# CEA-LIST/runia_core

Measured on AMD Instinct MI355X. Metric: OOD scores/sec, LaREM 16-MC PCA-256 (ResNet-18 layer4 latent 512x4x4), higher is better.
Workload: dtype f64

## Files before the change

include/runia_hip.h:

```cpp
#ifndef RUNIA_HIP_H
#define RUNIA_HIP_H

#include <stddef.h>
#include <stdint.h>

#ifdef __cplusplus
extern "C" {
#endif

#define RUNIA_OK 0
#define RUNIA_E_INVALID (-1)
#define RUNIA_E_LAUNCH (-2)
#define RUNIA_E_NODEVICE (-3)
#define RUNIA_E_WORKSPACE (-4)

typedef void* runia_stream_t;

int runia_abi_version(void);
const char* runia_error_string(int code);
int runia_device_count(void);
int runia_clock_probe(uint64_t* out4, int chain, runia_stream_t stream);
int runia_time_next_launch(void* start_event, void* stop_event);

int runia_mc_stack_f32(const float* x, const float* rand, int64_t rand_image_stride, float* out,
// ... 71 lines not shown

int runia_row_lse_msp_f32(const float* logits, float* lse, float* msp, int64_t N, int64_t C,
                          runia_stream_t stream);

int runia_l2_normalize_f32(const float* x, float* y, int64_t N, int64_t D, runia_stream_t stream);
size_t runia_knn_workspace_bytes(int64_t N, int64_t M, int64_t D, int k);
int runia_knn_piece_products(int64_t N, int64_t M, int64_t D);
size_t runia_knn_bank_state_bytes(int64_t M, int64_t D);
int runia_knn_prepare_bank_f32(const float* bank, void* state, size_t state_bytes, int64_t M, int64_t D,
                               runia_stream_t stream);
size_t runia_knn_prepared_workspace_bytes(int64_t N, int64_t M, int64_t D, int k);
int runia_knn_kth_prepared_f32(const float* q, const float* bank, const void* state, size_t state_bytes, float* score,
                               void* workspace, size_t workspace_bytes, int64_t N, int64_t M, int64_t D, int k,
                               runia_stream_t stream);
int runia_knn_kth_f32(const float* q, const float* bank, float* score, void* workspace,
                      size_t workspace_bytes, int64_t N, int64_t M, int64_t D, int k,
                      runia_stream_t stream);

int runia_kde_score_f64(const double* train, const double* x, double* score, int64_t M, int64_t N,
                        int64_t D, double bandwidth, runia_stream_t stream);
int runia_kde_score_kernel_f64(const double* train, const double* x, double* score, int64_t M, int64_t N, int64_t D,
                               double bandwidth, int kind, runia_stream_t stream);
int runia_row_sqnorm_f64(const double* x, double* out, int64_t N, int64_t D, runia_stream_t stream);
size_t runia_kde_workspace_bytes(int64_t N, int64_t M);
int runia_kde_score_packed_f64(const double* packed_train_t, const double* train_sqnorm, const double* x,
                               double* score, void* workspace, size_t workspace_bytes, int64_t M, int64_t N,
                               int64_t D, double bandwidth, runia_stream_t stream);

int runia_mc_entropy_supported(int H, int W, int n_mc, int k);
size_t runia_mc_entropy_workspace_bytes(int64_t N, int H, int W, int n_mc);
int runia_mc_mask_table_f32(const float* rand, int64_t rand_image_stride, void* workspace,
                            size_t workspace_bytes, int64_t N, int H, int W, int n_mc, double drop_prob,
                            int block_size, runia_stream_t stream);
int runia_mc_stack_table_f32(const float* x, const float* rand, int64_t rand_image_stride, float* z,
                             void* workspace, size_t workspace_bytes, int64_t N, int C, int H, int W, int n_mc,
                             double drop_prob, int block_size, runia_stream_t stream);
int runia_mc_entropy_from_table_f32(const float* x, const void* workspace, size_t workspace_bytes, double* h,
                                    float* z_out, double* zero_fill, int64_t N, int C, int H, int W, int n_mc,
                                    int k, double min_dist, runia_stream_t stream);
int runia_mc_entropy_f32(const float* x, const float* rand, int64_t rand_image_stride, double* h,
                         float* z_out, double* zero_fill, void* workspace, size_t workspace_bytes, int64_t N,
                         int C, int H, int W, int n_mc, double drop_prob, int block_size, int k, double min_dist,
                         runia_stream_t stream);
int runia_mc_draws_f32(float* out, int64_t N, int n_mc, int H, int W, uint64_t seed, int64_t first_image,
                       runia_stream_t stream);
int runia_mc_mask_table_counter_f32(uint64_t seed, int64_t first_image, void* workspace, size_t workspace_bytes,
                                    int64_t N, int H, int W, int n_mc, double drop_prob, int block_size,
                                    int redraw_dead_layers, runia_stream_t stream);
int runia_mc_entropy_counter_f32(const float* x, uint64_t seed, int64_t first_image, double* h, float* z_out,
                                 double* zero_fill, void* workspace, size_t workspace_bytes, int64_t N, int C, int H,
                                 int W, int n_mc, double drop_prob, int block_size, int k, double min_dist,
                                 int redraw_dead_layers, runia_stream_t stream);
int runia_pca_md_score_f64(const double* h, const double* packed_ct, const double* bias,
                           const double* scale, const double* md_mean, const double* packed_p,
                           double* score, double* y_out, int64_t N, int64_t D, int64_t n,
                           runia_stream_t stream);
size_t runia_proj_sq_workspace_bytes(int64_t N);
int runia_proj_sq_accumulate_f64(const double* h, const double* packed_m, const double* c, double* score,
                                 int64_t N, int64_t D, int64_t r, runia_stream_t stream);
int runia_proj_sq_score_f64(const double* h, const double* packed_m, const double* c, double* score,
                            void* workspace, size_t workspace_bytes, int64_t N, int64_t D, int64_t r,
                            runia_stream_t stream);
int runia_proj_sq_accumulate_trap_f64(const double* h, const double* packed_m, const double* c, double* score,
                                      int64_t N, int64_t D, int64_t r, runia_stream_t stream);
int runia_proj_sq_score_trap_f64(const double* h, const double* packed_m, const double* c, double* score,
                                 void* workspace, size_t workspace_bytes, int64_t N, int64_t D, int64_t r,
// ... 245 lines not shown
```

runia_core_amd/_hip.py:

```python
from __future__ import annotations

import contextlib
import ctypes
import os
import threading
from ctypes import c_char_p, c_double, c_float, c_int, c_int64, c_size_t, c_uint64, c_void_p
from typing import NamedTuple, Optional, Tuple, Union

import numpy as np
import torch

from . import config as _config

_LIB_PATH = os.path.join(os.path.dirname(os.path.abspath(__file__)), "librunia_hip.so")
_lib: Optional[ctypes.CDLL] = None

_SIGNATURES = {
    "runia_abi_version": (c_int, []),
    "runia_error_string": (c_char_p, [c_int]),
    "runia_device_count": (c_int, []),
    "runia_clock_probe": (c_int, [c_void_p, c_int, c_void_p]),
    "runia_time_next_launch": (c_int, [c_void_p, c_void_p]),
    "runia_mc_stack_f32": (
        c_int,
# ... 41 lines not shown
        c_int,
        [c_void_p, c_void_p, c_void_p, c_void_p, c_void_p, c_void_p, c_size_t, c_int64, c_int64, c_int, c_void_p],
    ),
    "runia_mahalanobis_score_f64": (
        c_int,
        [c_void_p, c_void_p, c_void_p, c_void_p, c_void_p, c_void_p, c_size_t, c_int64, c_int64, c_int, c_void_p],
    ),
    "runia_row_lse_msp_f32": (c_int, [c_void_p, c_void_p, c_void_p, c_int64, c_int64, c_void_p]),
    "runia_l2_normalize_f32": (c_int, [c_void_p, c_void_p, c_int64, c_int64, c_void_p]),
    "runia_kde_score_kernel_f64": (c_int, [c_void_p, c_void_p, c_void_p, c_int64, c_int64, c_int64, c_double, c_int, c_void_p]),
    "runia_knn_workspace_bytes": (c_size_t, [c_int64, c_int64, c_int64, c_int]),
    "runia_knn_piece_products": (c_int, [c_int64, c_int64, c_int64]),
    "runia_knn_bank_state_bytes": (c_size_t, [c_int64, c_int64]),
    "runia_knn_prepare_bank_f32": (c_int, [c_void_p, c_void_p, c_size_t, c_int64, c_int64, c_void_p]),
    "runia_knn_prepared_workspace_bytes": (c_size_t, [c_int64, c_int64, c_int64, c_int]),
    "runia_knn_kth_prepared_f32": (c_int, [c_void_p, c_void_p, c_void_p, c_size_t, c_void_p, c_void_p, c_size_t, c_int64, c_int64,
                                           c_int64, c_int, c_void_p]),
    "runia_knn_kth_f32": (
        c_int,
        [c_void_p, c_void_p, c_void_p, c_void_p, c_size_t, c_int64, c_int64, c_int64, c_int, c_void_p],
    ),
    "runia_kde_score_f64": (c_int, [c_void_p, c_void_p, c_void_p, c_int64, c_int64, c_int64, c_double, c_void_p]),
    "runia_row_sqnorm_f64": (c_int, [c_void_p, c_void_p, c_int64, c_int64, c_void_p]),
    "runia_kde_workspace_bytes": (c_size_t, [c_int64, c_int64]),
    "runia_kde_score_packed_f64": (
        c_int,
        [c_void_p, c_void_p, c_void_p, c_void_p, c_void_p, c_size_t, c_int64, c_int64, c_int64, c_double, c_void_p],
    ),
    "runia_mc_entropy_supported": (c_int, [c_int, c_int, c_int, c_int]),
    "runia_mc_entropy_workspace_bytes": (c_size_t, [c_int64, c_int, c_int, c_int]),
    "runia_mc_mask_table_f32": (
        c_int,
        [c_void_p, c_int64, c_void_p, c_size_t, c_int64, c_int, c_int, c_int, c_double, c_int, c_void_p],
    ),
    "runia_mc_stack_table_f32": (
        c_int,
        [c_void_p, c_void_p, c_int64, c_void_p, c_void_p, c_size_t, c_int64, c_int, c_int, c_int, c_int, c_double, c_int,
         c_void_p],
    ),
    "runia_mc_entropy_from_table_f32": (
        c_int,
        [c_void_p, c_void_p, c_size_t, c_void_p, c_void_p, c_void_p, c_int64, c_int, c_int, c_int, c_int, c_int,
         c_double, c_void_p],
    ),
    "runia_mc_entropy_f32": (
        c_int,
        [c_void_p, c_void_p, c_int64, c_void_p, c_void_p, c_void_p, c_void_p, c_size_t, c_int64, c_int, c_int, c_int,
         c_int, c_double, c_int, c_int, c_double, c_void_p],
    ),
    "runia_mc_draws_f32": (c_int, [c_void_p, c_int64, c_int, c_int, c_int, c_uint64, c_int64, c_void_p]),
    "runia_mc_mask_table_counter_f32": (
        c_int,
        [c_uint64, c_int64, c_void_p, c_size_t, c_int64, c_int, c_int, c_int, c_double, c_int, c_int, c_void_p],
    ),
    "runia_mc_entropy_counter_f32": (
        c_int,
        [c_void_p, c_uint64, c_int64, c_void_p, c_void_p, c_void_p, c_void_p, c_size_t, c_int64, c_int, c_int, c_int,
         c_int, c_double, c_int, c_int, c_double, c_int, c_void_p],
    ),
    "runia_select_hist_f32": (c_int, [c_void_p, c_void_p, c_int64, ctypes.c_uint32, ctypes.c_uint32, c_int, c_void_p]),
    "runia_cholesky_f32": (c_int, [c_void_p, c_void_p, c_int64, c_int64, c_double, c_void_p]),
    "runia_cholesky_f64": (c_int, [c_void_p, c_void_p, c_int64, c_int64, c_double, c_void_p]),
    "runia_gmm_log_prob_workspace_bytes": (c_size_t, [c_int64, c_int64, c_int]),
    "runia_gmm_log_prob_f32": (c_int, [c_void_p, c_void_p, c_void_p, c_void_p, c_void_p, c_void_p, c_void_p, c_size_t, c_int64,
                                       c_int64, c_int, c_void_p]),
    "runia_ood_metrics_workspace_bytes": (c_size_t, [c_int64]),
# ... 1056 lines not shown
def reserve_timed_events(n: int) -> None:
    pool = _TIMED_EVENT_POOL.setdefault(torch.cuda.current_device(), [])
    for _ in range(int(n)):
        e0, e1 = torch.cuda.Event(enable_timing=True), torch.cuda.Event(enable_timing=True)
        e0.record()
        e1.record()
        pool.append((e0, e1))


def _timed_launch_events():
    pool = _TIMED_EVENT_POOL.setdefault(torch.cuda.current_device(), [])
    if not pool:
        reserve_timed_events(1)
    e0, e1 = pool.pop()
    call("runia_time_next_launch", e0.cuda_event, e1.cuda_event)
    return e0, e1


def _timed_call(name: str, *args):
    e0, e1 = _timed_launch_events()
    try:
        launch(name, *args)
    finally:
        load_library().runia_time_next_launch(None, None)
    return e0, e1


def mc_entropy_supported(h: int, w: int, n_mc: int, k: int) -> bool:
    return bool(query("runia_mc_entropy_supported", int(h), int(w), int(n_mc), int(k)))


@_device_guard()
def mc_mask_table(rand: Union[torch.Tensor, CounterDraws, None], n: int, h: int, w: int, n_mc: int, drop_prob: float,
                  block_size: int, out: Optional[torch.Tensor] = None) -> torch.Tensor:
    lib = load_library()
    dev = require_gpu()
    assert 0 < n <= 65535
    ws_bytes = int(lib.runia_mc_entropy_workspace_bytes(n, h, w, n_mc))
    if out is None:
        out = torch.empty(max(ws_bytes, 16), dtype=torch.uint8, device=dev)
    assert out.is_cuda and out.dtype == torch.uint8 and out.numel() >= ws_bytes
    if isinstance(rand, CounterDraws):
        launch("runia_mc_mask_table_counter_f32", int(rand.seed) & (2**64 - 1), int(rand.first_image), out.data_ptr(), ws_bytes,
               n, h, w, n_mc, float(drop_prob), int(block_size), int(bool(rand.redraw_dead_layers)))
        return out
    rand, stride = _draws(rand, n, n_mc, h, w, copy=False)
    launch("runia_mc_mask_table_f32", _ptr(rand), stride, out.data_ptr(), ws_bytes, n, h, w, n_mc,
           float(drop_prob) if rand is not None else 0.0, int(block_size))
    return out


@_device_guard()
def mc_entropy(x: torch.Tensor, rand: Union[torch.Tensor, CounterDraws, None], n_mc: int, drop_prob: float, block_size: int, k: int,
               min_dist: float = 1e-5, want_samples: bool = False, out: Optional[torch.Tensor] = None,
               kernel_events: Optional[list] = None, zero_fill: Optional[torch.Tensor] = None,
               table: Optional[torch.Tensor] = None):
    lib = load_library()
    require_gpu()
    assert x.is_cuda and x.dtype == torch.float32 and x.dim() == 4
    x = x.contiguous()
    n, c, hh, ww = x.shape
    if table is not None:
        h = torch.empty((n, c), dtype=torch.float64, device=x.device) if out is None else out
        assert h.is_cuda and h.dtype == torch.float64 and h.shape == (n, c) and h.is_contiguous()
        z = torch.empty((n * n_mc, c), dtype=torch.float32, device=x.device) if want_samples else None
        ws_bytes = int(lib.runia_mc_entropy_workspace_bytes(n, hh, ww, n_mc))
        assert table.is_cuda and table.numel() >= ws_bytes and n <= 65535
        if zero_fill is not None:
            assert zero_fill.is_cuda and zero_fill.dtype == torch.float64 and zero_fill.shape == (n,) and zero_fill.is_contiguous()
        args = (x.data_ptr(), table.data_ptr(), ws_bytes, h.data_ptr(), _ptr(z), _ptr(zero_fill), n, c, hh, ww, n_mc, int(k),
                float(min_dist))
        if kernel_events is not None:
            kernel_events.append(_timed_call("runia_mc_entropy_from_table_f32", *args))
        else:
            launch("runia_mc_entropy_from_table_f32", *args)
        return (h, z) if want_samples else h
    counter = rand if isinstance(rand, CounterDraws) else None
    rand, stride = _draws(None if counter is not None else rand, n, n_mc, hh, ww)
    if out is None:
        h = torch.empty((n, c), dtype=torch.float64, device=x.device)
    else:
# ... 800 lines not shown
```

runia_core_amd/csrc/fused.hip:

```cpp
#include "common.hpp"
#include "entropy_core.hpp"
#include "mfma_f64_tile.hpp"
#include "philox.hpp"
#include "div_consts.hpp"
#include "trap_order.hpp"

namespace {

using namespace runia_entropy;
using namespace runia_mfma;

constexpr int kMaxMC = 64;
typedef float f2 __attribute__((ext_vector_type(2)));

__device__ __forceinline__ void layer_consts(int cnt, int& m, float& flag, float& zh, float& zl) {
  const int a = cnt ? __ffs(cnt) - 1 : 0;
  m = cnt >> a;
  flag = __uint_as_float((unsigned)(127 - a) << 23);
  zh = cnt ? __uint_as_float(runia_div::kDivHi[(m - 1) >> 1]) : NAN;
  zl = cnt ? __uint_as_float(runia_div::kDivLo[(m - 1) >> 1]) : 0.f;
}

__device__ __forceinline__ float add_f32(float a, float b) {
  float r;
// ... 4 lines not shown
__device__ __forceinline__ float div_newton(float u, float den, float r) {
  const float q = u * r;
  const float e = fmaf(-den, q, u);
  return fmaf(e, r, q);
}

template <int HT, int WT>
__host__ __device__ constexpr int mask_slot(int p) {
  if constexpr (HT % 2 == 0) {
    const int y = p / WT, xw = p - y * WT;
    return ((y >> 1) * WT + xw) * 2 + (y & 1);
  } else {
    return p;
  }
}

template <int HT, int WT>
__host__ __device__ constexpr int slot_position(int slot) {
  if constexpr (HT % 2 == 0) {
    const int e = slot & 1, t = slot >> 1;
    const int k = t / WT, xw = t - k * WT;
    return (2 * k + e) * WT + xw;
  } else {
    return slot;
  }
}

template <int HT, int WT>
__device__ __forceinline__ unsigned long long columns_below(int k) {
  unsigned long long row = (k >= 64) ? ~0ull : ((1ull << k) - 1ull), m = 0ull;
#pragma unroll
  for (int y = 0; y < HT; ++y) m |= row << (y * WT);
  return m;
}

constexpr int kMaskBitsWaves = 4;

template <int HT, int WT, int NP, bool REDRAW = false>
__global__ __launch_bounds__(64 * kMaskBitsWaves) void mc_mask_bits_kernel(const float* __restrict__ rnd,
                                                                           int64_t rand_stride,
                                                                           float* __restrict__ table, int64_t N,
                                                                           int n_mc, float gamma, int block_size,
                                                                           int identity, int sort_layers,
                                                                           uint64_t rng_seed, int64_t first_image) {
  constexpr int HW = HT * WT;
  static_assert(HW <= 64 && NP <= 64, "one drop layer per 64-bit word");
  constexpr bool DIV = (64 % HW == 0);
  constexpr int WORDS = (NP * HW + 63) / 64;
  constexpr unsigned long long FULL = (HW == 64) ? ~0ull : ((1ull << HW) - 1ull);
  const int lane = threadIdx.x & 63;
  const int64_t img = (int64_t)blockIdx.x * kMaskBitsWaves + (threadIdx.x >> 6);
  if (img >= N) return;
  const int bit0 = lane * HW, word0 = bit0 >> 6, off = bit0 & 63;
  const int pad = block_size / 2;

  auto seeds_of = [&](unsigned attempt) -> unsigned long long {
    float d[WORDS];
    if (rnd) {
      const float* r = rnd + img * rand_stride;
#pragma unroll
      for (int t = 0; t < WORDS; ++t) {
        const int i = lane + 64 * t;
        d[t] = (i < n_mc * HW) ? r[i] : 1.0f;
      }
    } else {
#pragma unroll
      for (int q = 0; q < (WORDS + 3) / 4; ++q) {
        const runia_philox::u4 b = runia_philox::lane_block(rng_seed, (uint64_t)(first_image + img), lane, q, attempt);
#pragma unroll
        for (int j = 0; j < 4; ++j) {
          const int t = 4 * q + j;
          if (t < WORDS) d[t] = (lane + 64 * t < n_mc * HW) ? runia_philox::component(b, j) : 1.0f;
        }
      }
    }
    unsigned long long lo = 0ull, hi = 0ull;
#pragma unroll
    for (int t = 0; t < WORDS; ++t) {
      const unsigned long long w = __ballot(d[t] < gamma);
      if (t == word0) lo = w;
      if (!DIV && t == word0 + 1) hi = w;
    }
    unsigned long long sd = lo >> off;
    if (!DIV && off + HW > 64) sd |= hi << (64 - off);
    return sd & FULL;
  };
  auto keep_of = [&](unsigned long long seed) -> unsigned long long {
    unsigned long long hx = 0ull;
    for (int dx = 0; dx < block_size; ++dx) {
      const int ox = dx - pad;
      if (ox >= WT || -ox >= WT) continue;
      hx |= (ox >= 0) ? ((seed >> ox) & columns_below<HT, WT>(WT - ox))
                      : ((seed << -ox) & ~columns_below<HT, WT>(-ox) & FULL);
    }
    unsigned long long dropped = 0ull;
    for (int dy = 0; dy < block_size; ++dy) {
      const int oy = dy - pad;
      if (oy >= HT || -oy >= HT) continue;
      dropped |= (oy >= 0) ? (hx >> (oy * WT)) : ((hx << (-oy * WT)) & FULL);
    }
    return ~dropped & FULL;
  };

  unsigned long long keep = identity ? FULL : keep_of(seeds_of(0u));
  if (REDRAW && !identity && !rnd) {
    for (unsigned attempt = 1; attempt <= 16u; ++attempt) {
      if (__ballot(lane < n_mc && keep == 0ull) == 0ull) break;
      const unsigned long long again = keep_of(seeds_of(attempt));
      if (keep == 0ull) keep = again;
    }
  }
  const int cnt = __popcll(keep);
  int m;
  float flag, zh, zl;
  layer_consts(cnt, m, flag, zh, zl);
  const int key = m ? m : 127;
  int rank = 0;
#pragma unroll
  for (int j = 0; j < NP; ++j) {
    const int o = __shfl(key, j, 64);
    rank += (j < n_mc) && ((o < key) || (o == key && j < lane));
  }
  if (!sort_layers) rank = lane;
  if (lane >= n_mc) return;
  float* out = table + img * (int64_t)(n_mc * (HW + 2));
  float* rec = out + rank * HW;
  if constexpr (HW % 4 == 0) {
#pragma unroll
    for (int c = 0; c < HW / 4; ++c) {
      float4 v;
      v.x = ((keep >> slot_position<HT, WT>(4 * c)) & 1ull) ? flag : 0.f;
      v.y = ((keep >> slot_position<HT, WT>(4 * c + 1)) & 1ull) ? flag : 0.f;
      v.z = ((keep >> slot_position<HT, WT>(4 * c + 2)) & 1ull) ? flag : 0.f;
      v.w = ((keep >> slot_position<HT, WT>(4 * c + 3)) & 1ull) ? flag : 0.f;
      reinterpret_cast<float4*>(rec)[c] = v;
    }
  } else {
#pragma unroll
    for (int q = 0; q < HW; ++q) rec[q] = ((keep >> slot_position<HT, WT>(q)) & 1ull) ? flag : 0.f;
  }
  out[n_mc * HW + rank] = zh;
  out[n_mc * (HW + 1) + rank] = zl;
}

#ifndef K1_BLOCK
#define K1_BLOCK 128
#endif
constexpr int kK1Block = K1_BLOCK;

struct RoiSource {
  const float* nhwc;
  const unsigned* table;
  int64_t image_bytes;
  int C;
  int roi_dwords;
};

template <int HT, int WT, int G>
__device__ __forceinline__ void roi_load_map(float (&u)[HT * WT], const RoiSource* __restrict__ src, int64_t roi, int c) {
  typedef const __attribute__((address_space(4))) unsigned* cptr;
  cptr tab = (cptr)(src->table + roi * (int64_t)src->roi_dwords);
  const unsigned image = tab[0];
  const __amdgpu_buffer_rsrc_t rsrc = __builtin_amdgcn_make_buffer_rsrc(
      const_cast<float*>(src->nhwc) + (int64_t)image * (src->image_bytes / 4), 0, (int)src->image_bytes, 0x00020000);
  const int voff = c * 4;
  cptr rows = tab + 8, cols = tab + 8 + 4 * (HT * G);
  constexpr float count = (float)(G * G);
  constexpr int SX = WT * G, SY = HT * G;
  unsigned ox_lo[SX], ox_hi[SX];
  float hx[SX], lx[SX];
#pragma unroll
  for (int sx = 0; sx < SX; ++sx) {
    ox_lo[sx] = cols[4 * sx];
    ox_hi[sx] = cols[4 * sx + 1];
    hx[sx] = __uint_as_float(cols[4 * sx + 2]);
// ... 345 lines not shown
      v += shfl_xor_f64(v, 1);
      v += shfl_xor_f64(v, 2);
      v += shfl_xor_f64(v, 4);
      v += shfl_xor_f64(v, 8);
      if (li == 0) part[wave * BM + 16 * a + lg + 4 * r] = v;
    }
  __syncthreads();
  if (tid < BM) {
    const int64_t row = r0 + tid;
    if (row < g.N) g.score[row] = -(((part[tid] + part[BM + tid]) + part[2 * BM + tid]) + part[3 * BM + tid]);
  }
}

struct ProjSqArgs {
  const double* h;
  const double* packed_m;
  const double* c;
  double* score;
  double* partial;
  int64_t N, D, r;
};

#ifndef K2_WAVES
#define K2_WAVES 5
#endif
#ifndef K2_DMA
#define K2_DMA 1
#endif
#ifndef K2_WAVES_DMA
#define K2_WAVES_DMA 5
#endif
#ifndef K2_TRAP_FORM
#define K2_TRAP_FORM 2
#endif
#ifndef K2_TRAP_ROT
#define K2_TRAP_ROT 2
#endif
#ifndef K2_TRAP_HALFMAP
#define K2_TRAP_HALFMAP 1
#endif
template <int RT, int NCT, bool ACCUMULATE, bool SPLIT, bool DMA, int TRAP = 0>
__global__ __launch_bounds__(256, (RT == 1 && NCT <= 2) ? (DMA ? K2_WAVES_DMA : K2_WAVES) : 1) void proj_sq_kernel(ProjSqArgs g) {
#if defined(__HIP_DEVICE_COMPILE__)
  constexpr int BM = 16 * RT;
  constexpr bool WAVE_SKIP = TRAP >= 2 && DMA && RT == 1;
  __shared__ double lds_a[DMA ? 1 : 2 * BM * APITCH];
  __shared__ __attribute__((aligned(16))) double lds_d0[DMA ? BM * KC : 2];
  __shared__ __attribute__((aligned(16))) double lds_d1[DMA ? BM * KC : 2];
  constexpr int NG = (NCT + 1) / 2;
  __shared__ double part[4 * NG * BM];
  const int64_t n_pad = n_padded(g.r);
  const int tid = threadIdx.x, lane = tid & 63;
  const int wave = __builtin_amdgcn_readfirstlane(tid >> 6);
  const int li = lane & 15, lg = lane >> 4;
  const int64_t NT = n_pad / 16;
  int64_t tile = blockIdx.x;
  int half = 0;
  if constexpr (SPLIT) {
    tile = (int64_t)(blockIdx.x >> 4) * 8 + (blockIdx.x & 7);
    const unsigned j = blockIdx.x >> 3;
    half = (int)((K2_TRAP_HALFMAP ? j ^ (j >> 5) : j) & 1);
    if (tile * BM >= g.N) return;
  }
  const int64_t r0 = tile * BM;
  const int nchunks = (int)(k_padded(g.D) / KC);
  const int rot = K2_TRAP_ROT == 1 ? (int)(tile & 3)
                  : K2_TRAP_ROT == 2 ? (int)(((blockIdx.x >> 4) + (blockIdx.x >> 8)) & 3)
                  : K2_TRAP_ROT == 3 ? (int)((blockIdx.x >> 8) & 3) : 0;
  const int grp = WAVE_SKIP ? (wave + rot) & 3 : wave;
  constexpr int PER_T = BM * KC / 256;
  double rowsq[NG][RT][4];
#pragma unroll
  for (int q = 0; q < NG; ++q)
#pragma unroll
    for (int a = 0; a < RT; ++a)
#pragma unroll
      for (int r = 0; r < 4; ++r) rowsq[q][a][r] = 0.0;
  for (int64_t cb = 0; cb < n_pad / BN; ++cb) {
    const int64_t ctbase = cb * 16 + (int64_t)half * (4 * NCT) + grp * NCT;
    int64_t wg_chunk = (cb * 16 + (int64_t)half * (4 * NCT)) * 16 / KC, wave_chunk = ctbase * 16 / KC;
    if constexpr (TRAP == 3) {
      const int64_t wg_pos = (cb * 16 + (int64_t)half * (4 * NCT)) / 2, wave_pos = ctbase / 2;
      wg_chunk = trap_balanced_first_k(wg_pos, g.r) / KC;
#pragma unroll
      for (int i = 1; i < 2 * NCT; ++i) {
        const int64_t f = trap_balanced_first_k(wg_pos + i, g.r) / KC;
        wg_chunk = f < wg_chunk ? f : wg_chunk;
      }
      wave_chunk = trap_balanced_first_k(wave_pos, g.r) / KC;
#pragma unroll
      for (int q = 1; q < NG; ++q) {
        const int64_t f = trap_balanced_first_k(wave_pos + q, g.r) / KC;
        wave_chunk = f < wave_chunk ? f : wave_chunk;
      }
    }
    const int ch0 = TRAP ? (int)(wg_chunk < nchunks - 1 ? wg_chunk : nchunks - 1) : 0;
    [[maybe_unused]] const int ws = WAVE_SKIP ? (int)(wave_chunk < nchunks - 1 ? wave_chunk : nchunks - 1) : ch0;
    d4 acc[RT][NCT];
#pragma unroll
    for (int a = 0; a < RT; ++a)
#pragma unroll
      for (int c = 0; c < NCT; ++c) acc[a][c] = (d4){0.0, 0.0, 0.0, 0.0};
    double2 bring[4][NCT];
    if constexpr (DMA) {
      const __amdgpu_buffer_rsrc_t brsrc = buffer_of(g.packed_m, (unsigned)(packed_elems(g.D, g.r) * 8));
      const int64_t rows_here = (g.N - r0 < BM) ? g.N - r0 : BM;
      const __amdgpu_buffer_rsrc_t arsrc = buffer_of(g.h + r0 * g.D, (unsigned)(rows_here * g.D * 8));
      const unsigned lane_bytes = (unsigned)lane * 16u;
      const unsigned pair_stride_bytes = (unsigned)NT * 1024u;
      const unsigned ct_bytes = (unsigned)ctbase * 1024u;
      constexpr int NDMA = BM / 4 / 4;
      unsigned a_lane_bytes[NDMA];
// ... 74 lines not shown
  #pragma unroll
        for (int q = 0; q < PER_T; ++q) lds_a[(buf * BM + srow + q * (256 / KC)) * APITCH + skk] = areg[q];
        __syncthreads();
        if (ch + 1 < nchunks) load_a((ch + 1) * KC);
        mfma_chunk_ring<RT, NCT>(acc, lds_a + buf * BM * APITCH, APITCH, li, lg, bp + (ch - ch0) * 4 * NT * 64, NT * 64, bring);
        buf ^= 1;
      }
    }
#pragma unroll
    for (int a = 0; a < RT; ++a)
#pragma unroll
      for (int c = 0; c < NCT; ++c) {
        const int64_t col = (ctbase + c) * 16 + li;
        const double cc = (col < g.r) ? g.c[col] : 0.0;
#pragma unroll
        for (int r = 0; r < 4; ++r) {
          const double v = acc[a][c][r] + cc;
          rowsq[c / 2][a][r] = fma(v, v, rowsq[c / 2][a][r]);
        }
      }
    __syncthreads();
  }
#pragma unroll
  for (int q = 0; q < NG; ++q)
#pragma unroll
    for (int a = 0; a < RT; ++a)
#pragma unroll
      for (int r = 0; r < 4; ++r) {
        double v = rowsq[q][a][r];
        v += shfl_xor_f64(v, 1);
        v += shfl_xor_f64(v, 2);
        v += shfl_xor_f64(v, 4);
        v += shfl_xor_f64(v, 8);
        if (li == 0) part[(grp * NG + q) * BM + 16 * a + lg + 4 * r] = v;
      }
  __syncthreads();
  if (tid < BM) {
    const int64_t row = r0 + tid;
    if (row < g.N) {
      const double lo = ((part[tid] + part[BM + tid]) + part[2 * BM + tid]) + part[3 * BM + tid];
      if constexpr (NCT == 4) {
        const double hi = ((part[4 * BM + tid] + part[5 * BM + tid]) + part[6 * BM + tid]) + part[7 * BM + tid];
        g.score[row] = -(lo + hi);
      } else if constexpr (!SPLIT) {
        if constexpr (ACCUMULATE) unsafeAtomicAdd(&g.score[row], -lo);
        else g.score[row] = -lo;
      } else if constexpr (ACCUMULATE) {
        unsafeAtomicAdd(&g.score[row], -lo);
      } else {
        g.partial[(int64_t)half * g.N + row] = lo;
      }
    }
  }
#endif
}

__global__ void proj_sq_combine_kernel(const double* __restrict__ partial, double* __restrict__ score, int64_t N) {
  const int64_t i = (int64_t)blockIdx.x * blockDim.x + threadIdx.x;
  if (i < N) score[i] = -(partial[i] + partial[N + i]);
}

double digamma_diff(int n, int k) {
  double s = 0.0;
  for (int j = n - 1; j >= k; --j) s += 1.0 / (double)j;
  return s;
}

// ... 3 lines not shown
  const int64_t n_pad = n_padded(g.n);
  const size_t shmem = ((size_t)2 * BM * APITCH + (size_t)BM * (n_pad + 2) + 4 * BM) * sizeof(double);
  if (shmem > 160 * 1024) return RUNIA_E_INVALID;
  static std::atomic<uint64_t> lds_ok{0};
  if (runia_allow_dynamic_lds(reinterpret_cast<const void*>(pca_md_kernel<RT>), 160 * 1024, lds_ok) != RUNIA_OK)
    return RUNIA_E_LAUNCH;
  const int64_t tiles = (g.N + BM - 1) / BM;
  pca_md_kernel<RT><<<(unsigned)tiles, 256, shmem, s>>>(g);
  return runia_check_launch();
}

}

extern "C" int runia_pca_md_score_f64(const double* h, const double* packed_ct, const double* bias,
                                      const double* scale, const double* md_mean, const double* packed_p,
                                      double* score, double* y_out, int64_t N, int64_t D, int64_t n,
                                      runia_stream_t stream) {
  if (N < 0 || D <= 0 || n <= 0) return RUNIA_E_INVALID;
  if (N == 0) return RUNIA_OK;
  if (!h || !md_mean || !packed_p || !score) return RUNIA_E_INVALID;
  if (packed_ct ? !bias : (n != D)) return RUNIA_E_INVALID;
  PcaMdArgs g{h, packed_ct, bias, scale, md_mean, packed_p, score, y_out, N, D, n};
  const int64_t tiles32 = (N + 31) / 32;
  const int64_t n_pad = n_padded(n);
  const bool fits32 = ((size_t)2 * 32 * APITCH + (size_t)32 * (n_pad + 2) + 128) * 8 <= 160 * 1024;
  if (tiles32 >= 1024 && fits32) return launch_pca_md<2>(g, as_stream(stream));
  return launch_pca_md<1>(g, as_stream(stream));
}

namespace {
template <int HH, int WW, int NPP>
void launch_mask(const float* rnd, int64_t rand_image_stride, float* table, int64_t N, int n_mc, float gamma,
                 int block_size, int identity, int sort_layers, uint64_t seed, int64_t first_image, int redraw,
                 hipStream_t s) {
  static_assert(HH * WW <= 64, "mc_mask_bits_kernel holds a drop layer in one 64-bit word");
  const unsigned grid = (unsigned)((N + kMaskBitsWaves - 1) / kMaskBitsWaves);
  if (redraw)
    mc_mask_bits_kernel<HH, WW, NPP, true><<<grid, 64 * kMaskBitsWaves, 0, s>>>(rnd, rand_image_stride, table, N, n_mc, gamma,
                                                                              block_size, identity, sort_layers, seed, first_image);
  else
    mc_mask_bits_kernel<HH, WW, NPP, false><<<grid, 64 * kMaskBitsWaves, 0, s>>>(rnd, rand_image_stride, table, N, n_mc, gamma,
                                                                               block_size, identity, sort_layers, seed, first_image);
}

__global__ void mc_draws_kernel(float* __restrict__ out, int64_t N, int per_image, uint64_t seed, int64_t first_image) {
  const int64_t i = (int64_t)blockIdx.x * blockDim.x + threadIdx.x;
  if (i >= N * per_image) return;
  const int64_t img = i / per_image;
  out[i] = runia_philox::draw(seed, (uint64_t)(first_image + img), (int)(i - img * per_image));
}
}

extern "C" int runia_mc_entropy_supported(int H, int W, int n_mc, int k);

extern "C" size_t runia_mc_entropy_workspace_bytes(int64_t N, int H, int W, int n_mc) {
  if (N <= 0 || H <= 0 || W <= 0 || n_mc <= 0) return 0;
  return (size_t)N * (size_t)n_mc * (size_t)(H * W + 2) * sizeof(float);
}

static int mc_args_ok(int64_t N, int H, int W, int n_mc, const void* workspace, size_t workspace_bytes) {
  if (N < 0 || N > 65535 || H <= 0 || W <= 0 || n_mc < 2 || n_mc > kMaxMC) return RUNIA_E_INVALID;
  if (N == 0) return RUNIA_OK;
  if (!workspace || workspace_bytes < runia_mc_entropy_workspace_bytes(N, H, W, n_mc) ||
      (((uintptr_t)workspace) & 15) != 0)
    return RUNIA_E_WORKSPACE;
  return RUNIA_OK;
}

#define RUNIA_MCE_SHAPES(F) \
  F(4, 4, 16, 5) F(4, 4, 32, 5) F(4, 4, 8, 5) F(2, 2, 16, 5) F(2, 2, 32, 5) F(7, 7, 16, 5) F(7, 7, 32, 5) F(8, 8, 16, 5) F(8, 8, 32, 5)

static int mc_mask_table(const float* rnd, int64_t rand_image_stride, void* workspace, size_t workspace_bytes,
                         int64_t N, int H, int W, int n_mc, double drop_prob, int block_size, int sort_layers,
                         runia_stream_t stream, bool counter = false, uint64_t seed = 0, int64_t first_image = 0,
                         int redraw = 0) {
  if (block_size < 1) return RUNIA_E_INVALID;
  if (int rc = mc_args_ok(N, H, W, n_mc, workspace, workspace_bytes)) return rc;
  if (N == 0) return RUNIA_OK;
  const int identity = (drop_prob == 0.0);
  if (!identity && !rnd && !counter) return RUNIA_E_INVALID;
  if (counter) rnd = nullptr;
  float* table = reinterpret_cast<float*>(workspace);
  const float gamma = (float)(drop_prob / (double)(block_size * block_size));
  hipStream_t s = as_stream(stream);
#define RUNIA_MCE(HH, WW, NPP, KK)                                                                          \
  if (H == HH && W == WW && n_mc <= NPP && n_mc > NPP / 2) {                                                \
    launch_mask<HH, WW, NPP>(rnd, rand_image_stride, table, N, n_mc, gamma, block_size, identity,           \
                             sort_layers, seed, first_image, redraw, s);                                    \
    return runia_check_launch();                                                                            \
  }
  RUNIA_MCE_SHAPES(RUNIA_MCE)
#undef RUNIA_MCE
  return RUNIA_E_INVALID;
}

extern "C" int runia_mc_mask_table_f32(const float* rnd, int64_t rand_image_stride, void* workspace,
                                       size_t workspace_bytes, int64_t N, int H, int W, int n_mc, double drop_prob,
                                       int block_size, runia_stream_t stream) {
  return mc_mask_table(rnd, rand_image_stride, workspace, workspace_bytes, N, H, W, n_mc, drop_prob, block_size, 1,
                       stream);
}

extern "C" int runia_mc_stack_table_f32(const float* x, const float* rnd, int64_t rand_image_stride, float* z,
                                        void* workspace, size_t workspace_bytes, int64_t N, int C, int H, int W,
                                        int n_mc, double drop_prob, int block_size, runia_stream_t stream) {
  if (C <= 0) return RUNIA_E_INVALID;
  if (int rc = mc_args_ok(N, H, W, n_mc, workspace, workspace_bytes)) return rc;
  if (N == 0) return RUNIA_OK;
  if (!x || !z || !runia_mc_entropy_supported(H, W, n_mc, 5)) return RUNIA_E_INVALID;
  if (!(((((uintptr_t)x) & 15) == 0) || (H * W) % 4 != 0)) return RUNIA_E_INVALID;
  if (int rc = mc_mask_table(rnd, rand_image_stride, workspace, workspace_bytes, N, H, W, n_mc, drop_prob,
                             block_size, 0, stream))
    return rc;
  const float* table = reinterpret_cast<const float*>(workspace);
  const unsigned grid = (unsigned)((((N + 7) / 8 + K1_IMGS - 1) / K1_IMGS) * 8 * ((C + kK1Block - 1) / kK1Block));
  hipStream_t s = as_stream(stream);
#define RUNIA_MCE(HH, WW, NPP, KK)                                                                          \
  if (H == HH && W == WW && n_mc <= NPP && n_mc > NPP / 2) {                                                \
    if (n_mc == NPP)                                                                                        \
      mc_entropy_kernel<HH, WW, NPP, KK, true, false><<<grid, kK1Block, 0, s>>>(x, table, nullptr, z,       \
                                                                                nullptr, N, C, n_mc, 0.0,   \
                                                                                0.0, 0.0);                  \
    else                                                                                                    \
      mc_entropy_kernel<HH, WW, NPP, KK, false, false><<<grid, kK1Block, 0, s>>>(x, table, nullptr, z,      \
                                                                                 nullptr, N, C, n_mc, 0.0,  \
                                                                                 0.0, 0.0);                 \
    return runia_check_launch();                                                                            \
  }
  RUNIA_MCE_SHAPES(RUNIA_MCE)
#undef RUNIA_MCE
  return RUNIA_E_INVALID;
}

// ... 262 lines not shown
```

Measured before the change: 60.33 million.

## Add packed multi-image mask-table kernel for small spatial maps

Adds a mask-table kernel that packs several images into one wavefront, each lane owning one MC layer. It applies when H*W is 4 or 16 and the explicit draws are 16-byte aligned. It loads draws with float4, builds a 32-bit seed, and ranks layers with width-NP shuffles, instead of one image per wavefront with mostly idle lanes. The packed form becomes the default whenever it applies. Separately, the K2 trap kernel's wave-rotation option is removed and waves index directly.

```diff
diff --git a/include/runia_hip.h b/include/runia_hip.h
--- a/include/runia_hip.h
+++ b/include/runia_hip.h
@@ -127,6 +127,9 @@
 int runia_mc_mask_table_f32(const float* rand, int64_t rand_image_stride, void* workspace,
                             size_t workspace_bytes, int64_t N, int H, int W, int n_mc, double drop_prob,
                             int block_size, runia_stream_t stream);
+int runia_mc_mask_table_form_f32(const float* rand, int64_t rand_image_stride, void* workspace,
+                                 size_t workspace_bytes, int64_t N, int H, int W, int n_mc, double drop_prob,
+                                 int block_size, int sort_layers, int form, runia_stream_t stream);
 int runia_mc_stack_table_f32(const float* x, const float* rand, int64_t rand_image_stride, float* z,
                              void* workspace, size_t workspace_bytes, int64_t N, int C, int H, int W, int n_mc,
                              double drop_prob, int block_size, runia_stream_t stream);
diff --git a/runia_core_amd/_hip.py b/runia_core_amd/_hip.py
--- a/runia_core_amd/_hip.py
+++ b/runia_core_amd/_hip.py
@@ -97,6 +97,10 @@
     "runia_mc_mask_table_f32": (
         c_int,
         [c_void_p, c_int64, c_void_p, c_size_t, c_int64, c_int, c_int, c_int, c_double, c_int, c_void_p],
+    ),
+    "runia_mc_mask_table_form_f32": (
+        c_int,
+        [c_void_p, c_int64, c_void_p, c_size_t, c_int64, c_int, c_int, c_int, c_double, c_int, c_int, c_int, c_void_p],
     ),
     "runia_mc_stack_table_f32": (
         c_int,
@@ -1219,7 +1223,8 @@
 
 @_device_guard()
 def mc_mask_table(rand: Union[torch.Tensor, CounterDraws, None], n: int, h: int, w: int, n_mc: int, drop_prob: float,
-                  block_size: int, out: Optional[torch.Tensor] = None) -> torch.Tensor:
+                  block_size: int, out: Optional[torch.Tensor] = None, form: Optional[int] = None,
+                  sort_layers: bool = True) -> torch.Tensor:
     lib = load_library()
     dev = require_gpu()
     assert 0 < n <= 65535
@@ -1228,12 +1233,19 @@
         out = torch.empty(max(ws_bytes, 16), dtype=torch.uint8, device=dev)
     assert out.is_cuda and out.dtype == torch.uint8 and out.numel() >= ws_bytes
     if isinstance(rand, CounterDraws):
+        if form is not None or not sort_layers:
+            raise ValueError("form= and sort_layers= choose among the kernels for explicit draws")
         launch("runia_mc_mask_table_counter_f32", int(rand.seed) & (2**64 - 1), int(rand.first_image), out.data_ptr(), ws_bytes,
                n, h, w, n_mc, float(drop_prob), int(block_size), int(bool(rand.redraw_dead_layers)))
         return out
     rand, stride = _draws(rand, n, n_mc, h, w, copy=False)
-    launch("runia_mc_mask_table_f32", _ptr(rand), stride, out.data_ptr(), ws_bytes, n, h, w, n_mc,
-           float(drop_prob) if rand is not None else 0.0, int(block_size))
+    if form is None and sort_layers:
+        launch("runia_mc_mask_table_f32", _ptr(rand), stride, out.data_ptr(), ws_bytes, n, h, w, n_mc,
+               float(drop_prob) if rand is not None else 0.0, int(block_size))
+    else:
+        launch("runia_mc_mask_table_form_f32", _ptr(rand), stride, out.data_ptr(), ws_bytes, n, h, w, n_mc,
+               float(drop_prob) if rand is not None else 0.0, int(block_size), int(bool(sort_layers)),
+               -1 if form is None else int(form))
     return out
 
 
diff --git a/runia_core_amd/csrc/fused.hip b/runia_core_amd/csrc/fused.hip
--- a/runia_core_amd/csrc/fused.hip
+++ b/runia_core_amd/csrc/fused.hip
@@ -60,6 +60,49 @@
 #pragma unroll
   for (int y = 0; y < HT; ++y) m |= row << (y * WT);
   return m;
+}
+
+template <int HT, int WT, typename Word>
+__device__ __forceinline__ Word keep_of(Word seed, int block_size) {
+  constexpr Word FULL = (HT * WT == 64) ? (Word)~0ull : (Word)((1ull << (HT * WT)) - 1ull);
+  const int pad = block_size / 2;
+  Word hx = 0;
+  for (int dx = 0; dx < block_size; ++dx) {
+    const int ox = dx - pad;
+    if (ox >= WT || -ox >= WT) continue;
+    hx |= (ox >= 0) ? ((seed >> ox) & (Word)columns_below<HT, WT>(WT - ox))
+                    : ((seed << -ox) & (Word)~columns_below<HT, WT>(-ox) & FULL);
+  }
+  Word dropped = 0;
+  for (int dy = 0; dy < block_size; ++dy) {
+    const int oy = dy - pad;
+    if (oy >= HT || -oy >= HT) continue;
+    dropped |= (oy >= 0) ? (hx >> (oy * WT)) : ((hx << (-oy * WT)) & FULL);
+  }
+  return ~dropped & FULL;
+}
+
+template <int HT, int WT, typename Word>
+__device__ __forceinline__ void store_record(float* __restrict__ out, int rank, int n_mc, Word keep, float flag,
+                                             float zh, float zl) {
+  constexpr int HW = HT * WT;
+  float* rec = out + rank * HW;
+  if constexpr (HW % 4 == 0) {
+#pragma unroll
+    for (int c = 0; c < HW / 4; ++c) {
+      float4 v;
+      v.x = ((keep >> slot_position<HT, WT>(4 * c)) & 1) ? flag : 0.f;
+      v.y = ((keep >> slot_position<HT, WT>(4 * c + 1)) & 1) ? flag : 0.f;
+      v.z = ((keep >> slot_position<HT, WT>(4 * c + 2)) & 1) ? flag : 0.f;
+      v.w = ((keep >> slot_position<HT, WT>(4 * c + 3)) & 1) ? flag : 0.f;
+      reinterpret_cast<float4*>(rec)[c] = v;
+    }
+  } else {
+#pragma unroll
+    for (int q = 0; q < HW; ++q) rec[q] = ((keep >> slot_position<HT, WT>(q)) & 1) ? flag : 0.f;
+  }
+  out[n_mc * HW + rank] = zh;
+  out[n_mc * (HW + 1) + rank] = zl;
 }
 
 constexpr int kMaskBitsWaves = 4;
@@ -80,7 +123,6 @@
   const int64_t img = (int64_t)blockIdx.x * kMaskBitsWaves + (threadIdx.x >> 6);
   if (img >= N) return;
   const int bit0 = lane * HW, word0 = bit0 >> 6, off = bit0 & 63;
-  const int pad = block_size / 2;
 
   auto seeds_of = [&](unsigned attempt) -> unsigned long long {
     float d[WORDS];
@@ -113,28 +155,12 @@
     if (!DIV && off + HW > 64) sd |= hi << (64 - off);
     return sd & FULL;
   };
-  auto keep_of = [&](unsigned long long seed) -> unsigned long long {
-    unsigned long long hx = 0ull;
-    for (int dx = 0; dx < block_size; ++dx) {
-      const int ox = dx - pad;
-      if (ox >= WT || -ox >= WT) continue;
-      hx |= (ox >= 0) ? ((seed >> ox) & columns_below<HT, WT>(WT - ox))
-                      : ((seed << -ox) & ~columns_below<HT, WT>(-ox) & FULL);
-    }
-    unsigned long long dropped = 0ull;
-    for (int dy = 0; dy < block_size; ++dy) {
-      const int oy = dy - pad;
-      if (oy >= HT || -oy >= HT) continue;
-      dropped |= (oy >= 0) ? (hx >> (oy * WT)) : ((hx << (-oy * WT)) & FULL);
-    }
-    return ~dropped & FULL;
-  };
-
-  unsigned long long keep = identity ? FULL : keep_of(seeds_of(0u));
+
+  unsigned long long keep = identity ? FULL : keep_of<HT, WT>(seeds_of(0u), block_size);
   if (REDRAW && !identity && !rnd) {
     for (unsigned attempt = 1; attempt <= 16u; ++attempt) {
       if (__ballot(lane < n_mc && keep == 0ull) == 0ull) break;
-      const unsigned long long again = keep_of(seeds_of(attempt));
+      const unsigned long long again = keep_of<HT, WT>(seeds_of(attempt), block_size);
       if (keep == 0ull) keep = again;
     }
   }
@@ -151,24 +177,48 @@
   }
   if (!sort_layers) rank = lane;
   if (lane >= n_mc) return;
-  float* out = table + img * (int64_t)(n_mc * (HW + 2));
-  float* rec = out + rank * HW;
-  if constexpr (HW % 4 == 0) {
-#pragma unroll
-    for (int c = 0; c < HW / 4; ++c) {
-      float4 v;
-      v.x = ((keep >> slot_position<HT, WT>(4 * c)) & 1ull) ? flag : 0.f;
-      v.y = ((keep >> slot_position<HT, WT>(4 * c + 1)) & 1ull) ? flag : 0.f;
-      v.z = ((keep >> slot_position<HT, WT>(4 * c + 2)) & 1ull) ? flag : 0.f;
-      v.w = ((keep >> slot_position<HT, WT>(4 * c + 3)) & 1ull) ? flag : 0.f;
-      reinterpret_cast<float4*>(rec)[c] = v;
-    }
-  } else {
-#pragma unroll
-    for (int q = 0; q < HW; ++q) rec[q] = ((keep >> slot_position<HT, WT>(q)) & 1ull) ? flag : 0.f;
-  }
-  out[n_mc * HW + rank] = zh;
-  out[n_mc * (HW + 1) + rank] = zl;
+  store_record<HT, WT>(table + img * (int64_t)(n_mc * (HW + 2)), rank, n_mc, keep, flag, zh, zl);
+}
+
+template <int HT, int WT, int NP>
+__global__ __launch_bounds__(64 * kMaskBitsWaves) void mc_mask_packed_kernel(const float* __restrict__ rnd,
+                                                                             int64_t rand_stride,
+                                                                             float* __restrict__ table, int64_t N,
+                                                                             int n_mc, float gamma, int block_size,
+                                                                             int identity, int sort_layers) {
+  constexpr int HW = HT * WT, IMGS = 64 / NP;
+  static_assert(HW % 4 == 0 && HW <= 32 && 64 % NP == 0, "a layer is a few 16-byte loads and one 32-bit word");
+  constexpr unsigned FULL = (1u << HW) - 1u;
+  const int lane = threadIdx.x & 63, layer = lane % NP;
+  const int64_t img0 = ((int64_t)blockIdx.x * kMaskBitsWaves + (threadIdx.x >> 6)) * IMGS;
+  if (img0 >= N) return;
+  const int64_t img = img0 + lane / NP;
+  const bool live = img < N && layer < n_mc;
+  unsigned keep = FULL;
+  if (!identity) {
+    unsigned seed = 0u;
+    if (live) {
+      const float4* r = reinterpret_cast<const float4*>(rnd + img * rand_stride + layer * HW);
+#pragma unroll
+      for (int c = 0; c < HW / 4; ++c) {
+        const float4 d = r[c];
+        seed |= (unsigned)(d.x < gamma) << (4 * c) | (unsigned)(d.y < gamma) << (4 * c + 1) |
+                (unsigned)(d.z < gamma) << (4 * c + 2) | (unsigned)(d.w < gamma) << (4 * c + 3);
+      }
+    }
+    keep = keep_of<HT, WT>(seed, block_size);
+  }
+  const int cnt = __popc(keep);
+  int m;
+  float flag, zh, zl;
+  layer_consts(cnt, m, flag, zh, zl);
+  const int key = live ? ((m ? m : 127) << 6 | layer) : 0x7fffffff;
+  int rank = 0;
+#pragma unroll
+  for (int j = 0; j < NP; ++j) rank += __shfl(key, j, NP) < key;
+  if (!sort_layers) rank = layer;
+  if (!live) return;
+  store_record<HT, WT>(table + img * (int64_t)(n_mc * (HW + 2)), rank, n_mc, keep, flag, zh, zl);
 }
 
 #ifndef K1_BLOCK
@@ -580,9 +630,6 @@
 #endif
 #ifndef K2_TRAP_FORM
 #define K2_TRAP_FORM 2
-#endif
-#ifndef K2_TRAP_ROT
-#define K2_TRAP_ROT 2
 #endif
 #ifndef K2_TRAP_HALFMAP
 #define K2_TRAP_HALFMAP 1
@@ -612,10 +659,6 @@
   }
   const int64_t r0 = tile * BM;
   const int nchunks = (int)(k_padded(g.D) / KC);
-  const int rot = K2_TRAP_ROT == 1 ? (int)(tile & 3)
-                  : K2_TRAP_ROT == 2 ? (int)(((blockIdx.x >> 4) + (blockIdx.x >> 8)) & 3)
-                  : K2_TRAP_ROT == 3 ? (int)((blockIdx.x >> 8) & 3) : 0;
-  const int grp = WAVE_SKIP ? (wave + rot) & 3 : wave;
   constexpr int PER_T = BM * KC / 256;
   double rowsq[NG][RT][4];
 #pragma unroll
@@ -625,7 +668,7 @@
 #pragma unroll
       for (int r = 0; r < 4; ++r) rowsq[q][a][r] = 0.0;
   for (int64_t cb = 0; cb < n_pad / BN; ++cb) {
-    const int64_t ctbase = cb * 16 + (int64_t)half * (4 * NCT) + grp * NCT;
+    const int64_t ctbase = cb * 16 + (int64_t)half * (4 * NCT) + wave * NCT;
     int64_t wg_chunk = (cb * 16 + (int64_t)half * (4 * NCT)) * 16 / KC, wave_chunk = ctbase * 16 / KC;
     if constexpr (TRAP == 3) {
       const int64_t wg_pos = (cb * 16 + (int64_t)half * (4 * NCT)) / 2, wave_pos = ctbase / 2;
@@ -766,7 +809,7 @@
         v += shfl_xor_f64(v, 2);
         v += shfl_xor_f64(v, 4);
         v += shfl_xor_f64(v, 8);
-        if (li == 0) part[(grp * NG + q) * BM + 16 * a + lg + 4 * r] = v;
+        if (li == 0) part[(wave * NG + q) * BM + 16 * a + lg + 4 * r] = v;
       }
   __syncthreads();
   if (tid < BM) {
@@ -836,8 +879,16 @@
 template <int HH, int WW, int NPP>
 void launch_mask(const float* rnd, int64_t rand_image_stride, float* table, int64_t N, int n_mc, float gamma,
                  int block_size, int identity, int sort_layers, uint64_t seed, int64_t first_image, int redraw,
-                 hipStream_t s) {
+                 bool packed, hipStream_t s) {
   static_assert(HH * WW <= 64, "mc_mask_bits_kernel holds a drop layer in one 64-bit word");
+  if constexpr (HH * WW == 4 || HH * WW == 16) {
+    if (packed) {
+      constexpr int per_wg = kMaskBitsWaves * (64 / NPP);
+      mc_mask_packed_kernel<HH, WW, NPP><<<(unsigned)((N + per_wg - 1) / per_wg), 64 * kMaskBitsWaves, 0, s>>>(
+          rnd, rand_image_stride, table, N, n_mc, gamma, block_size, identity, sort_layers);
+      return;
+    }
+  }
   const unsigned grid = (unsigned)((N + kMaskBitsWaves - 1) / kMaskBitsWaves);
   if (redraw)
     mc_mask_bits_kernel<HH, WW, NPP, true><<<grid, 64 * kMaskBitsWaves, 0, s>>>(rnd, rand_image_stride, table, N, n_mc, gamma,
@@ -877,20 +928,24 @@
 static int mc_mask_table(const float* rnd, int64_t rand_image_stride, void* workspace, size_t workspace_bytes,
                          int64_t N, int H, int W, int n_mc, double drop_prob, int block_size, int sort_layers,
                          runia_stream_t stream, bool counter = false, uint64_t seed = 0, int64_t first_image = 0,
-                         int redraw = 0) {
-  if (block_size < 1) return RUNIA_E_INVALID;
+                         int redraw = 0, int form = -1) {
+  if (block_size < 1 || form < -1 || form > 1) return RUNIA_E_INVALID;
   if (int rc = mc_args_ok(N, H, W, n_mc, workspace, workspace_bytes)) return rc;
+  if (counter) rnd = nullptr;
+  const bool can_pack = rnd && !redraw && (H * W == 4 || H * W == 16) && n_mc <= 32 &&
+                        (((uintptr_t)rnd) & 15) == 0 && rand_image_stride % 4 == 0;
+  if (form == 1 && !can_pack) return RUNIA_E_INVALID;
+  const bool packed = form < 0 ? can_pack : (form == 1);
   if (N == 0) return RUNIA_OK;
   const int identity = (drop_prob == 0.0);
   if (!identity && !rnd && !counter) return RUNIA_E_INVALID;
-  if (counter) rnd = nullptr;
   float* table = reinterpret_cast<float*>(workspace);
   const float gamma = (float)(drop_prob / (double)(block_size * block_size));
   hipStream_t s = as_stream(stream);
 #define RUNIA_MCE(HH, WW, NPP, KK)                                                                          \
   if (H == HH && W == WW && n_mc <= NPP && n_mc > NPP / 2) {                                                \
     launch_mask<HH, WW, NPP>(rnd, rand_image_stride, table, N, n_mc, gamma, block_size, identity,           \
-                             sort_layers, seed, first_image, redraw, s);                                    \
+                             sort_layers, seed, first_image, redraw, packed, s);                            \
     return runia_check_launch();                                                                            \
   }
   RUNIA_MCE_SHAPES(RUNIA_MCE)
@@ -903,6 +958,14 @@
                                        int block_size, runia_stream_t stream) {
   return mc_mask_table(rnd, rand_image_stride, workspace, workspace_bytes, N, H, W, n_mc, drop_prob, block_size, 1,
                        stream);
+}
+
+extern "C" int runia_mc_mask_table_form_f32(const float* rnd, int64_t rand_image_stride, void* workspace,
+                                            size_t workspace_bytes, int64_t N, int H, int W, int n_mc,
+                                            double drop_prob, int block_size, int sort_layers, int form,
+                                            runia_stream_t stream) {
+  return mc_mask_table(rnd, rand_image_stride, workspace, workspace_bytes, N, H, W, n_mc, drop_prob, block_size,
+                       sort_layers ? 1 : 0, stream, false, 0, 0, 0, form);
 }
 
 extern "C" int runia_mc_stack_table_f32(const float* x, const float* rnd, int64_t rand_image_stride, float* z,
```

After: 61.15 million (median of 6 runs). 1.01x the previous value.
